# jnvance/DMRG.x

Hardware: NVIDIA B200
Metric: superblock H*psi algorithmic GB/s (higher is better)
Workload: dtype f64

## Files before the change

### dmrg.x_b200/csrc/abi.cpp

```cpp
#include <cstring>
#include <string>

#include "../../include/dmrgx.h"
#include <cmath>

#include "common.h"
#include "plan.h"

using namespace dmrgx;

namespace {
thread_local std::string g_msg;
template <class F>
int guard(F&& f) {
    try { f(); return 0; }
    catch (const Err& e) { g_msg = e.what(); return e.code ? e.code : 1; }
    catch (const std::exception& e) { g_msg = e.what(); return 1; }
    catch (...) { g_msg = "unknown error"; return 1; }
}
inline Ctx* cur(Ctx* c) { if (c && c->st) dev::make_current(c->st); return c; }
inline Ctx* C(dmrgx_ctx c) { return cur((Ctx*)c); }
inline Block* B(dmrgx_block b) { if (b) cur(((Block*)b)->ctx); return (Block*)b; }
inline Kron* K(dmrgx_kron k) { if (k) cur(((Kron*)k)->ctx); return (Kron*)k; }
inline HShell* H(dmrgx_hshell h) { if (h) cur(((HShell*)h)->ctx); return (HShell*)h; }
// ... 107 lines not shown
    *out = nullptr;
    return guard([&] { *out = (dmrgx_hshell)hshell_create(K(k), terms_of(nterms, a, iop, isite, jop, jsite)); });
}
int dmrgx_hshell_create_single(dmrgx_kron k, int opl, dmrgx_int il, int opr, dmrgx_int ir, dmrgx_hshell* out) {
    *out = nullptr;
    return guard([&] { *out = (dmrgx_hshell)hshell_create_single(K(k), opl, (int)il, opr, (int)ir); });
}
int dmrgx_hshell_create_product(dmrgx_kron k, dmrgx_int nl, const int* lop, const dmrgx_int* lsite, dmrgx_int nr, const int* rop,
                                const dmrgx_int* rsite, dmrgx_hshell* out) {
    *out = nullptr;
    return guard([&] {
        std::vector<std::pair<int, int>> l, r;
        for (dmrgx_int i = 0; i < nl; ++i) l.push_back({lop[i], (int)lsite[i]});
        for (dmrgx_int i = 0; i < nr; ++i) r.push_back({rop[i], (int)rsite[i]});
        *out = (dmrgx_hshell)hshell_create_product(K(k), l, r);
    });
}
int dmrgx_hshell_apply(dmrgx_hshell h, const double* d_x, double* d_y) { return guard([&] { hshell_apply(H(h), d_x, d_y); }); }
int dmrgx_hshell_apply_sharded(dmrgx_hshell h, double* d_x, double* d_y) { return guard([&] { hshell_apply_sharded(H(h), d_x, d_y); }); }
int dmrgx_hshell_halo_bytes(dmrgx_hshell h, double* halo, double* allgather) {
    HShell* s = H(h);
    if (halo) *halo = 8.0 * (double)s->halo_recv_elems;
    if (allgather) *allgather = 8.0 * (double)(s->n - (s->row_end - s->row_begin)) * (s->ctx->world > 1 ? 1.0 : 0.0);
    return 0;
}
int dmrgx_hshell_row_range(dmrgx_hshell h, dmrgx_int* begin, dmrgx_int* end, dmrgx_int* cuts) {
    HShell* s = H(h);
    if (begin) *begin = s->row_begin;
    if (end) *end = s->row_end;
    if (cuts) for (size_t i = 0; i < s->row_cuts.size(); ++i) cuts[i] = s->row_cuts[i];
    return 0;
}
int dmrgx_hshell_apply_stage(dmrgx_hshell h, int stage, const double* d_x, double* d_y) {
    return guard([&] {
        HShell* s = H(h);
        if (s->sparse) { if (stage == 2) hshell_apply(s, d_x, d_y); else if (stage != 1) throw Err(ERR_ARG_WRONG, "stage must be 1 or 2"); return; }
        if (stage == 1) s->stage1.run(s->ctx, d_x, nullptr);
        else if (stage == 2) s->stage2.run(s->ctx, d_x, d_y);
        else throw Err(ERR_ARG_WRONG, "stage must be 1 or 2");
    });
}
int dmrgx_hshell_stage_flops(dmrgx_hshell h, double* flops1, double* flops2) {
    *flops1 = H(h)->stage1.flops; *flops2 = H(h)->stage2.flops;
    return 0;
}
dmrgx_int dmrgx_hshell_plan_items(dmrgx_hshell h, int stage, dmrgx_int cap, dmrgx_int* out4) {
    const Plan& p = stage == 1 ? H(h)->stage1 : H(h)->stage2;
    dmrgx_int n = 0;
    for (const dev::WorkItem& it : p.items) {
        if (n < cap) {
            long long ks = 0;
            for (int sgi = it.seg_begin; sgi < it.seg_end; ++sgi) if (p.segs[sgi].type == dev::SEG_GEMM) ks += p.segs[sgi].K;
            out4[4 * n] = it.tm; out4[4 * n + 1] = it.tn; out4[4 * n + 2] = it.seg_end - it.seg_begin; out4[4 * n + 3] = ks;
        }
        ++n;
    }
    return n;
}
int dmrgx_hshell_plan_segtypes(dmrgx_hshell h, int stage, dmrgx_int* out6) {
    const Plan& p = stage == 1 ? H(h)->stage1 : H(h)->stage2;
    for (int i = 0; i < 6; ++i) out6[i] = 0;
    for (const dev::WorkItem& it : p.items)
        for (int sgi = it.seg_begin; sgi < it.seg_end; ++sgi) out6[p.segs[sgi].type]++;
    return 0;
}
int dmrgx_hshell_stage_exec_flops(dmrgx_hshell h, double* flops1, double* flops2) {
    *flops1 = H(h)->stage1.exec_flops; *flops2 = H(h)->stage2.exec_flops;
    return 0;
}
int dmrgx_hshell_apply_host(dmrgx_hshell h, const double* x, double* y) {
    return guard([&] {
        HShell* s = H(h);
        Ctx* ctx = s->ctx;
        const size_t bytes = (size_t)s->n * 8;
        if (!s->xbuf) {
            s->xbuf = std::make_shared<DevBuf>(ctx, bytes);
            s->ybuf = std::make_shared<DevBuf>(ctx, bytes);
        }
        const size_t lbytes = (size_t)(s->row_end - s->row_begin) * 8;
        dev::h2d(ctx->st, s->xbuf->as<double>() + s->row_begin, x, lbytes);
        hshell_apply_sharded(s, s->xbuf->as<double>(), s->ybuf->as<double>());
        dev::d2h(ctx->st, y, s->ybuf->as<double>() + s->row_begin, lbytes);
        dev::sync(ctx->st);
    });
}
int dmrgx_hshell_destroy(dmrgx_hshell h) { return guard([&] { if (h) { dev::sync(H(h)->ctx->st); delete H(h); } }); }
int dmrgx_hshell_workspace_bytes(dmrgx_hshell h, double* bytes) {
    HShell* s = H(h);
    double b = 16.0 * (double)s->n + (s->work ? (double)s->work->bytes : 0.0);
    for (const BufRef& k : s->keep) b += (double)k->bytes;
    *bytes = b;
    return 0;
}
int dmrgx_hshell_stats_global(dmrgx_hshell h, double* alg_bytes, double* alg_flops) {
    *alg_bytes = (double)H(h)->alg_bytes_global; *alg_flops = H(h)->alg_flops_global;
    return 0;
}
int dmrgx_hshell_stats(dmrgx_hshell h, dmrgx_int* nstates, dmrgx_int* nterms, double* alg_bytes, double* alg_flops, dmrgx_int* nt1, dmrgx_int* nt2) {
    HShell* s = H(h);
    if (nstates) *nstates = s->n;
    if (nterms) *nterms = s->nterms;
    if (alg_bytes) *alg_bytes = (double)s->alg_bytes;
    if (alg_flops) *alg_flops = s->alg_flops;
    if (nt1) *nt1 = (dmrgx_int)s->stage1.items.size();
    if (nt2) *nt2 = s->sparse ? (dmrgx_int)s->sparse->tiles.size() : (dmrgx_int)s->stage2.items.size();
    return 0;
// ... 201 lines not shown
```

### dmrg.x_b200/csrc/dev.h

```cpp
#pragma once
#include <cstddef>
#include <cstdint>

namespace dev {

enum SegType : int { SEG_GEMM = 0, SEG_AXPY = 1, SEG_DIAG = 2, SEG_CSRA = 3, SEG_CSRB = 4, SEG_CSRADD = 5 };

struct Segment {
    const double* A;
    const double* B;
    const int* rowptr;
    const int* colidx;
    long long lda_m, lda_k;
    long long ldb_n, ldb_k;
    double coef;
    int K;
    int type;
    int row0;
    int d;
    int flags;
    int pad;
};
enum : int { SEGF_A_X = 1, SEGF_B_X = 2 };

struct WorkItem {
    double* C;
    long long ldc;
    int m0, n0;
    int tm, tn;
    int seg_begin, seg_end;
    int mode;
    int c_in_y;
};

constexpr int TILE = 64;

struct Stream;

int init(int device, void* user_stream, Stream** out);
void destroy(Stream*);
const char* last_error();
void make_current(Stream*);

void* malloc_bytes(Stream*, size_t bytes);
void free_bytes(Stream*, void* p);
void h2d(Stream*, void* dst, const void* src, size_t bytes);
void d2h(Stream*, void* dst, const void* src, size_t bytes);
void d2d(Stream*, void* dst, const void* src, size_t bytes);
void memset0(Stream*, void* dst, size_t bytes);
void sync(Stream*);
long long launch_count();

constexpr int COMM_ID_BYTES = 128;
int comm_unique_id(void* out);
int comm_init(Stream*, int rank, int world, const void* id);
void allreduce_sum(Stream*, double* d_buf, long long n);
void allgatherv(Stream*, double* d_buf, const long long* offsets);
void exchange_ranges(Stream*, double* d_buf, int n, const int* from, const int* to, const long long* off, const long long* cnt);
void bcast_batch(Stream*, int n, double* const* d_ptr, const long long* count, const int* root);

void run_chain(Stream*, const WorkItem* d_items, int nitems, const Segment* d_segs, const double* x, double* y, double* w = nullptr);

constexpr int SP_ROWS = 4;
struct SpASlot { long long src[SP_ROWS]; double w[SP_ROWS]; };
struct SpSSlot { int roff[SP_ROWS]; int pad[SP_ROWS]; double w[SP_ROWS]; };
struct SpBSlot { const int* ecol; const double* eval; int W, ld; int all_in, pad; int roff[SP_ROWS]; long long src[SP_ROWS]; double w[SP_ROWS]; };
struct SpTile {
    long long off;
    int nR, nrows;
    int a_begin, a_count;
    int s_begin, s_count;
    int b_begin, b_count;
    int pad[6];
};
constexpr int SP_MAX_NR = 3072;
void run_spmm(Stream*, const SpTile* d_tiles, int ntiles, const SpASlot* d_aslots, const SpSSlot* d_sslots, const SpBSlot* d_bslots, const double* x, double* y,
              int max_nR);

struct ReduceItem {
    double* dst;
    long long ldc;
    long long src_off;
    int tm, tn;
    int nparts;
    int dst_in_y;
};
void run_reduce(Stream*, const ReduceItem* d_items, int nitems, double* y, const double* w);

// ... 18 lines not shown
```

### dmrg.x_b200/csrc/dev_cuda.cu

```cuda
#include <cuda_runtime.h>
#include <dlfcn.h>
#include <nccl.h>

#include <chrono>
#include <map>
#include <unordered_map>
#include <cstdio>
#include <cstring>
#include <algorithm>
#include <stdexcept>
#include <string>
#include <vector>

#include "dev.h"

namespace dev {

static thread_local std::string g_err;
static long long g_launches = 0;
const char* last_error() { return g_err.c_str(); }
long long launch_count() { return g_launches; }

#define CUDA_OK(call)                                                                                   \
    do {                                                                                                \
// ... 175 lines not shown
}

template <bool MK>
struct Stager {
    const double* base;
    int off[8];
    long long kstep;
    int soff;
    int k0;
    unsigned rowmask;
    static constexpr int SI = MK ? 8 * S_MK : 2 * S_KM;
    __device__ __forceinline__ void init(const double* b, long long ld_row, long long ld_k, int ext, int tid) {
        base = b;
        if (MK) {
            const int k = tid & 15, r0 = tid >> 4;
            rowmask = 0;
#pragma unroll
            for (int i = 0; i < 8; ++i) {
                int r = r0 + 8 * i;
                if (r < ext) rowmask |= 1u << i;
                r = r < ext ? r : ext - 1;
                off[i] = (int)(r * ld_row + k * ld_k);
            }
            soff = r0 * S_MK + k;
            k0 = k;
        } else {
            const int r = tid & 63, kk = tid >> 6;
            const int rc = r < ext ? r : ext - 1;
            rowmask = r < ext ? 0xffu : 0u;
#pragma unroll
            for (int i = 0; i < 8; ++i) off[i] = (int)(rc * ld_row + (kk + 2 * i) * ld_k);
            soff = kk * S_KM + r;
            k0 = kk;
        }
        kstep = (long long)BK * ld_k;
    }
    template <bool ALLROWS>
    __device__ __forceinline__ void issue(double* sm, int krem) {
        if (krem >= BK) {
#pragma unroll
            for (int i = 0; i < 8; ++i)
                if (ALLROWS || ((rowmask >> i) & 1u)) cp_async8_all(sm + soff + i * SI, base + off[i]);
        } else {
#pragma unroll
            for (int i = 0; i < 8; ++i) {
                const bool v = (MK ? k0 : k0 + 2 * i) < krem;
                if (ALLROWS || ((rowmask >> i) & 1u)) cp_async8(sm + soff + i * SI, v ? base + off[i] : base, v);
            }
        }
        base += kstep;
    }
};

template <bool A_MK, bool B_NK, bool UNIT, int NMI, int NNI, int NKK = BK / 4>
__device__ __forceinline__ void chunk_mma(double (&acc)[4][4][2], const double* as, const double* bs, double coef) {
    constexpr int a_sm = A_MK ? S_MK : 1, a_sk = A_MK ? 1 : S_KM;
    constexpr int b_sn = B_NK ? S_MK : 1, b_sk = B_NK ? 1 : S_KM;
#pragma unroll
    for (int kk = 0; kk < NKK; ++kk) {
        double a[NMI], b[NNI];
#pragma unroll
        for (int mi = 0; mi < NMI; ++mi) a[mi] = as[mi * 8 * a_sm + kk * 4 * a_sk];
#pragma unroll
        for (int ni = 0; ni < NNI; ++ni) b[ni] = UNIT ? bs[ni * 8 * b_sn + kk * 4 * b_sk] : bs[ni * 8 * b_sn + kk * 4 * b_sk] * coef;
#pragma unroll
        for (int ni = 0; ni < NNI; ++ni)
#pragma unroll
            for (int mi = 0; mi < NMI; ++mi) dmma_m8n8k4(acc[mi][ni][0], acc[mi][ni][1], a[mi], b[ni]);
    }
}

template <int NSTAGE, bool A_MK, bool B_NK, bool FULL, bool UNIT>
__device__ __forceinline__ void gemm_segment(double (&acc)[4][4][2], const Segment& sg, const WorkItem& it, double* As, double* Bs,
                                             int tid, int rbase, int cbase, int g, int t, int nmi, int nni) {
    Stager<A_MK> sa;
    Stager<B_NK> sb;
    sa.init(sg.A + (long long)it.m0 * sg.lda_m, sg.lda_m, sg.lda_k, it.tm, tid);
    sb.init(sg.B + (long long)it.n0 * sg.ldb_n, sg.ldb_n, sg.ldb_k, it.tn, tid);
    const int K = sg.K;
    const int nchunks = (K + BK - 1) / BK;
    const double coef = sg.coef;
    constexpr int a_sm = A_MK ? S_MK : 1, a_sk = A_MK ? 1 : S_KM;
    constexpr int b_sn = B_NK ? S_MK : 1, b_sk = B_NK ? 1 : S_KM;
    const int a_base = (rbase + g) * a_sm + t * a_sk;
    const int b_base = (cbase + g) * b_sn + t * b_sk;
    __syncthreads();
#pragma unroll
    for (int p = 0; p < NSTAGE - 1; ++p) {
        if (p < nchunks) {
            sa.template issue<FULL>(As + p * SMEM_TILE, K - p * BK);
            sb.template issue<FULL>(Bs + p * SMEM_TILE, K - p * BK);
        }
        cp_async_commit();
    }
    int cur = 0, nxt = NSTAGE - 1;
    for (int c = 0; c < nchunks; ++c) {
        if (c + NSTAGE - 1 < nchunks) {
            const int krem = K - (c + NSTAGE - 1) * BK;
            sa.template issue<FULL>(As + nxt * SMEM_TILE, krem);
            sb.template issue<FULL>(Bs + nxt * SMEM_TILE, krem);
        }
        cp_async_commit();
        cp_async_wait<NSTAGE - 1>();
        __syncthreads();
        const double* as = As + cur * SMEM_TILE + a_base;
        const double* bs = Bs + cur * SMEM_TILE + b_base;
        if (FULL) {
            const int krem = K - c * BK;
            if (krem > 12) chunk_mma<A_MK, B_NK, UNIT, 4, 4, 4>(acc, as, bs, coef);
            else if (krem > 8) chunk_mma<A_MK, B_NK, UNIT, 4, 4, 3>(acc, as, bs, coef);
            else if (krem > 4) chunk_mma<A_MK, B_NK, UNIT, 4, 4, 2>(acc, as, bs, coef);
            else chunk_mma<A_MK, B_NK, UNIT, 4, 4, 1>(acc, as, bs, coef);
        } else {
#define MMA_CASE(M_, N_) case (M_) * 5 + (N_): chunk_mma<A_MK, B_NK, UNIT, M_, N_>(acc, as, bs, coef); break;
            switch (nmi * 5 + nni) {
                MMA_CASE(4, 4) MMA_CASE(4, 3) MMA_CASE(4, 2) MMA_CASE(4, 1)
                MMA_CASE(3, 4) MMA_CASE(3, 3) MMA_CASE(3, 2) MMA_CASE(3, 1)
                MMA_CASE(2, 4) MMA_CASE(2, 3) MMA_CASE(2, 2) MMA_CASE(2, 1)
                MMA_CASE(1, 4) MMA_CASE(1, 3) MMA_CASE(1, 2) MMA_CASE(1, 1)
                default: break;
            }
#undef MMA_CASE
        }
        __syncthreads();
        cur = cur + 1 == NSTAGE ? 0 : cur + 1;
        nxt = nxt + 1 == NSTAGE ? 0 : nxt + 1;
    }
}

template <int NSTAGE, bool A_MK, bool B_NK>
__device__ __forceinline__ void gemm_dispatch(double (&acc)[4][4][2], const Segment& sg, const WorkItem& it, double* As, double* Bs,
                                              int tid, int rbase, int cbase, int g, int t, int nmi, int nni) {
    if (sg.coef == 1.0) {
        if (it.tm == BM && it.tn == BM) gemm_segment<NSTAGE, A_MK, B_NK, true, true>(acc, sg, it, As, Bs, tid, rbase, cbase, g, t, 4, 4);
        else gemm_segment<NSTAGE, A_MK, B_NK, false, true>(acc, sg, it, As, Bs, tid, rbase, cbase, g, t, nmi, nni);
    } else gemm_segment<NSTAGE, A_MK, B_NK, false, false>(acc, sg, it, As, Bs, tid, rbase, cbase, g, t, nmi, nni);
}

template <int NSTAGE>
__global__ void __launch_bounds__(NTHREADS, 3) chain_kernel(const WorkItem* __restrict__ items, const Segment* __restrict__ segs,
                                                            const double* __restrict__ xbase, double* __restrict__ ybase,
                                                            double* __restrict__ wbase) {
    extern __shared__ __align__(16) double chain_smem[];
    double* As = chain_smem;
    double* Bs = chain_smem + NSTAGE * SMEM_TILE;
    WorkItem it = items[blockIdx.x];
    if (it.c_in_y) it.C = (double*)((char*)(it.c_in_y == 1 ? ybase : wbase) + (size_t)it.C);
    const int tid = threadIdx.x;
    const int warp = tid >> 5, lane = tid & 31;
    const int wm = warp >> 1, wn = warp & 1;
    const int g = lane >> 2, t = lane & 3;
    const int tm = it.tm, tn = it.tn;
    const int hm = ((tm + 15) >> 4) << 3, hn = ((tn + 15) >> 4) << 3;
    const int rbase = wm * hm, cbase = wn * hn;
    int nmi = (tm - rbase + 7) / 8; nmi = nmi < 0 ? 0 : (nmi > (hm >> 3) ? (hm >> 3) : nmi);
    int nni = (tn - cbase + 7) / 8; nni = nni < 0 ? 0 : (nni > (hn >> 3) ? (hn >> 3) : nni);

    double acc[4][4][2];
#pragma unroll
    for (int mi = 0; mi < 4; ++mi)
#pragma unroll
        for (int ni = 0; ni < 4; ++ni) { acc[mi][ni][0] = 0.0; acc[mi][ni][1] = 0.0; }

    for (int s = it.seg_begin; s < it.seg_end; ++s) {
        Segment sg = segs[s];
        if (sg.flags & SEGF_A_X) sg.A = (const double*)((const char*)xbase + (size_t)sg.A);
        if (sg.flags & SEGF_B_X) sg.B = (const double*)((const char*)xbase + (size_t)sg.B);
        if (sg.type == SEG_GEMM) {
            const bool a_mk = (sg.lda_k == 1) || (sg.lda_m != 1);
            const bool b_nk = (sg.ldb_k == 1) || (sg.ldb_n != 1);
            if (a_mk) {
                if (b_nk) gemm_dispatch<NSTAGE, true, true>(acc, sg, it, As, Bs, tid, rbase, cbase, g, t, nmi, nni);
                else gemm_dispatch<NSTAGE, true, false>(acc, sg, it, As, Bs, tid, rbase, cbase, g, t, nmi, nni);
            } else {
                if (b_nk) gemm_dispatch<NSTAGE, false, true>(acc, sg, it, As, Bs, tid, rbase, cbase, g, t, nmi, nni);
                else gemm_dispatch<NSTAGE, false, false>(acc, sg, it, As, Bs, tid, rbase, cbase, g, t, nmi, nni);
            }
        } else if (sg.type == SEG_AXPY) {
            const double* base = sg.A + (long long)(it.m0 + rbase + g) * sg.lda_m + (long long)(it.n0 + cbase + 2 * t) * sg.lda_k;
            const long long sm8 = 8 * sg.lda_m, sn8 = 8 * sg.lda_k, sn1 = sg.lda_k;
            double v[4][4][2];
#pragma unroll
            for (int mi = 0; mi < 4; ++mi) {
                const bool rok = mi < nmi && rbase + mi * 8 + g < tm;
#pragma unroll
                for (int ni = 0; ni < 4; ++ni) {
                    const int col = cbase + ni * 8 + 2 * t;
                    const bool c0 = rok && ni < nni && col < tn, c1 = rok && ni < nni && col + 1 < tn;
                    const double* q = base + mi * sm8 + ni * sn8;
                    v[mi][ni][0] = c0 ? q[0] : 0.0;
                    v[mi][ni][1] = c1 ? q[sn1] : 0.0;
                }
            }
            const double coef = sg.coef;
#pragma unroll
            for (int mi = 0; mi < 4; ++mi)
#pragma unroll
                for (int ni = 0; ni < 4; ++ni) { acc[mi][ni][0] += coef * v[mi][ni][0]; acc[mi][ni][1] += coef * v[mi][ni][1]; }
        } else if (sg.type == SEG_CSRA) {
            const double* xb = sg.A + (long long)(it.n0 + cbase + 2 * t) * sg.ldb_n;
#pragma unroll
            for (int mi = 0; mi < 4; ++mi) {
                const int row = rbase + mi * 8 + g;
                if (mi >= nmi || row >= tm) continue;
                const int r = sg.row0 + it.m0 + row;
                const int e1 = sg.rowptr[r + 1];
                for (int e = sg.rowptr[r]; e < e1; ++e) {
                    const double v = sg.B[e] * sg.coef;
                    const double* xr = xb + (long long)sg.colidx[e] * sg.ldb_k;
// ... 7 lines not shown
            }
        } else if (sg.type == SEG_CSRB) {
            const double* vb = sg.A + (long long)(it.m0 + rbase + g) * sg.lda_m;
#pragma unroll
            for (int ni = 0; ni < 4; ++ni) {
#pragma unroll
                for (int h = 0; h < 2; ++h) {
                    const int col = cbase + ni * 8 + 2 * t + h;
                    if (ni >= nni || col >= tn) continue;
                    const int r = sg.row0 + it.n0 + col;
                    const int e1 = sg.rowptr[r + 1];
                    for (int e = sg.rowptr[r]; e < e1; ++e) {
                        const double v = sg.B[e] * sg.coef;
                        const double* vc = vb + (long long)sg.colidx[e] * sg.lda_k;
#pragma unroll
                        for (int mi = 0; mi < 4; ++mi)
                            if (mi < nmi && rbase + mi * 8 + g < tm) acc[mi][ni][h] += v * vc[(long long)(mi * 8) * sg.lda_m];
                    }
                }
            }
        } else if (sg.type == SEG_CSRADD) {
#pragma unroll
            for (int mi = 0; mi < 4; ++mi) {
                const int row = rbase + mi * 8 + g;
                if (mi >= nmi || row >= tm) continue;
                const int r = sg.row0 + it.m0 + row;
                const int e1 = sg.rowptr[r + 1];
                for (int e = sg.rowptr[r]; e < e1; ++e) {
                    const int lc = sg.colidx[e] - sg.d - it.n0 - cbase - 2 * t;
                    const double v = sg.B[e] * sg.coef;
#pragma unroll
                    for (int ni = 0; ni < 4; ++ni) {
                        const int col = cbase + ni * 8 + 2 * t;
                        if (ni < nni && lc == ni * 8 && col < tn) acc[mi][ni][0] += v;
                        if (ni < nni && lc == ni * 8 + 1 && col + 1 < tn) acc[mi][ni][1] += v;
                    }
                }
            }
        } else if (sg.type == SEG_DIAG) {
#pragma unroll
            for (int mi = 0; mi < 4; ++mi) {
                const int row = rbase + mi * 8 + g;
                if (mi >= nmi || row >= tm) continue;
#pragma unroll
                for (int ni = 0; ni < 4; ++ni)
#pragma unroll
                    for (int h = 0; h < 2; ++h) {
                        const int col = cbase + ni * 8 + 2 * t + h;
                        if (ni < nni && col < tn && it.m0 + row + sg.d == it.n0 + col) acc[mi][ni][h] += sg.coef;
                    }
            }
        }
    }
#pragma unroll
    for (int mi = 0; mi < 4; ++mi) {
        const int row = rbase + mi * 8 + g;
        if (mi >= nmi || row >= tm) continue;
#pragma unroll
        for (int ni = 0; ni < 4; ++ni) {
#pragma unroll
            for (int h = 0; h < 2; ++h) {
                const int col = cbase + ni * 8 + 2 * t + h;
                if (ni >= nni || col >= tn) continue;
                double* p = it.C + (long long)row * it.ldc + col;
                if (it.mode == 0) *p = acc[mi][ni][h];
                else atomicAdd(p, acc[mi][ni][h]);
            }
        }
    }
}

void run_chain(Stream* st, const WorkItem* d_items, int nitems, const Segment* d_segs, const double* x, double* y, double* w) {
    if (nitems <= 0) return;
    constexpr int smem2 = 2 * 2 * SMEM_TILE * (int)sizeof(double), smem3 = 2 * 3 * SMEM_TILE * (int)sizeof(double);
    if (!st->chain_cfg) {
        CUDA_OK(cudaFuncSetAttribute(chain_kernel<3>, cudaFuncAttributeMaxDynamicSharedMemorySize, smem3));
        st->chain_cfg = true;
    }
    constexpr int deep_below = 1800;
    if (nitems < deep_below) chain_kernel<3><<<nitems, NTHREADS, smem3, st->s>>>(d_items, d_segs, x, y, w);
    else chain_kernel<2><<<nitems, NTHREADS, smem2, st->s>>>(d_items, d_segs, x, y, w);
    LAUNCH_CHECK();
}

constexpr int SP_BD = 256, SP_CH = 4, SP_AMAX = 24, SP_BMAX = 8;

__device__ __forceinline__ unsigned smem_u32(const void* p) { return (unsigned)__cvta_generic_to_shared(p); }
__device__ __forceinline__ void mbar_init(unsigned long long* b, int count) {
    asm volatile("mbarrier.init.shared::cta.b64 [%0], %1;\n" ::"r"(smem_u32(b)), "r"(count));
    asm volatile("fence.mbarrier_init.release.cluster;\n" ::: "memory");
}
__device__ __forceinline__ void mbar_expect_tx(unsigned long long* b, unsigned bytes) {
    asm volatile("mbarrier.arrive.expect_tx.shared::cta.b64 _, [%0], %1;\n" ::"r"(smem_u32(b)), "r"(bytes) : "memory");
}
__device__ __forceinline__ void bulk_g2s(void* dst, const void* src, unsigned bytes, unsigned long long* b) {
    asm volatile("cp.async.bulk.shared::cluster.global.mbarrier::complete_tx::bytes [%0], [%1], %2, [%3];\n" ::"r"(smem_u32(dst)), "l"(src), "r"(bytes),
                 "r"(smem_u32(b))
                 : "memory");
}
__device__ __forceinline__ void mbar_wait(unsigned long long* b, unsigned parity) {
    unsigned ok;
    do {
        asm volatile("{\n.reg .pred p;\nmbarrier.try_wait.parity.shared::cta.b64 p, [%1], %2;\nselp.u32 %0, 1, 0, p;\n}\n" : "=r"(ok) : "r"(smem_u32(b)), "r"(parity) : "memory");
    } while (!ok);
}

template <class T>
__device__ __forceinline__ void sp_stage(T* dst, const T* src, int count, int tid) {
    for (int i = tid; i < count * (int)(sizeof(T) / 8); i += SP_BD) ((double*)dst)[i] = __ldg((const double*)src + i);
}

__global__ void __launch_bounds__(SP_BD, 3) spmm_kernel(const SpTile* __restrict__ tiles, const SpASlot* __restrict__ aslots, const SpSSlot* __restrict__ sslots,
                                                       const SpBSlot* __restrict__ bslots, const double* __restrict__ x, double* __restrict__ y) {
    extern __shared__ __align__(16) unsigned char sp_smem[];
    __shared__ unsigned long long mbar;
    __shared__ SpTile s_tile;
// ... 1118 lines not shown
    const int max_sweeps = 40;
    while (!live.empty()) {
        const int nl = (int)live.size();
        int* sub_prefix = h_tab.data();
        int* app_prefix = h_tab.data() + nl + 1;
        sub_prefix[0] = 0; app_prefix[0] = 0;
        int maxnb = 0;
        for (int q = 0; q < nl; ++q) {
            const EigJob& jb = jobs[(size_t)live[(size_t)q]];
            ljobs[(size_t)q] = jb;
            const int npair = jb.nb / 2;
            sub_prefix[q + 1] = sub_prefix[q] + npair;
            app_prefix[q + 1] = app_prefix[q] + npair * (npair - 1) / 2 + npair * (jb.np / ET);
            maxnb = std::max(maxnb, jb.nb);
        }
        CUDA_OK(cudaMemcpyAsync(d_live, ljobs.data(), (size_t)nl * sizeof(EigJob), cudaMemcpyHostToDevice, st->s));
        CUDA_OK(cudaMemcpyAsync(d_tab, h_tab.data(), (size_t)(2 * nl + 2) * 4, cudaMemcpyHostToDevice, st->s));
        CUDA_OK(cudaStreamSynchronize(st->s));
        for (int rr = 0; rr < maxnb - 1; ++rr, ++round) {
            eig_sub_kernel<<<sub_prefix[nl], ESUB_THREADS, sub_smem, st->s>>>(d_live, d_tab, nl, round, sweeps_done == 0);
            LAUNCH_CHECK();
            eig_apply_kernel<<<app_prefix[nl], 128, app_smem, st->s>>>(d_live, d_tab + nl + 1, nl, round);
            LAUNCH_CHECK();
        }
        ++sweeps_done;
        for (int q = 0; q < nl; ++q) CUDA_OK(cudaMemcpyAsync(&h_active[(size_t)q], jobs[(size_t)live[(size_t)q]].active, 4, cudaMemcpyDeviceToHost, st->s));
        CUDA_OK(cudaStreamSynchronize(st->s));
        std::vector<int> next;
        for (int q = 0; q < nl; ++q) if (h_active[(size_t)q]) next.push_back(live[(size_t)q]);
        for (int q : next) CUDA_OK(cudaMemsetAsync(jobs[(size_t)q].active, 0, 4, st->s));
        live.swap(next);
        if (round > max_sweeps * 256 || (round / std::max(1, maxnb - 1)) > max_sweeps) { if (!live.empty()) { g_err = "block Jacobi did not converge"; rc = 107; } break; }
    }
    WorkItem* d_items = nullptr;
    Segment* d_segs = nullptr;
    if (!rc) {
        std::vector<WorkItem> items;
        std::vector<Segment> segs;
        for (int q = 0; q < nj; ++q) {
            const EigJob& jb = jobs[(size_t)q];
            Segment sg;
            std::memset(&sg, 0, sizeof sg);
            sg.type = SEG_GEMM; sg.coef = 1.0; sg.K = jb.n;
            sg.A = jb.VT; sg.lda_m = jb.np; sg.lda_k = 1;
            sg.B = jb.outA; sg.ldb_n = 1; sg.ldb_k = jb.n;
            segs.push_back(sg);
            for (int m0 = 0; m0 < jb.n; m0 += TILE)
                for (int n0 = 0; n0 < jb.n; n0 += TILE) {
                    WorkItem it;
                    std::memset(&it, 0, sizeof it);
                    it.C = jb.A + (long long)m0 * jb.np + n0; it.ldc = jb.np; it.m0 = m0; it.n0 = n0;
                    it.tm = std::min(TILE, jb.n - m0); it.tn = std::min(TILE, jb.n - n0);
                    it.seg_begin = q; it.seg_end = q + 1;
                    items.push_back(it);
                }
        }
        d_items = (WorkItem*)malloc_bytes(st, items.size() * sizeof(WorkItem));
        d_segs = (Segment*)malloc_bytes(st, segs.size() * sizeof(Segment));
        CUDA_OK(cudaMemcpyAsync(d_items, items.data(), items.size() * sizeof(WorkItem), cudaMemcpyHostToDevice, st->s));
        CUDA_OK(cudaMemcpyAsync(d_segs, segs.data(), segs.size() * sizeof(Segment), cudaMemcpyHostToDevice, st->s));
        for (int q = 0; q < nj; ++q) h_tab[(size_t)q] = (int)lam_off[(size_t)q];
        CUDA_OK(cudaMemcpyAsync(d_tab, rank_off.data(), (size_t)nj * 4, cudaMemcpyHostToDevice, st->s));
        CUDA_OK(cudaMemcpyAsync(d_tab + nj, h_tab.data(), (size_t)nj * 4, cudaMemcpyHostToDevice, st->s));
        run_chain(st, d_items, (int)items.size(), d_segs, nullptr, nullptr, nullptr);
        eig_rq_kernel<<<dim3(16, nj), 256, 0, st->s>>>(d_jobs, wd, d_tab + nj);
        LAUNCH_CHECK();
        eig_finish_kernel<<<dim3(4, nj), 256, 0, st->s>>>(d_jobs, wd, d_tab + nj, wi, d_tab);
        LAUNCH_CHECK();
        eig_gather_kernel<<<dim3(64, nj), 256, 0, st->s>>>(d_jobs, wi, d_tab);
        LAUNCH_CHECK();
        CUDA_OK(cudaStreamSynchronize(st->s));
    }
    join();
    CUDA_OK(cudaStreamSynchronize(st->s));
    free_bytes(st, d_items);
    free_bytes(st, d_segs);
    free_bytes(st, d_live);
    free_bytes(st, d_jobs);
    free_bytes(st, wi);
    free_bytes(st, wd);
    return rc;
}

}
```

### dmrg.x_b200/csrc/plan.cpp

```cpp
#include <algorithm>
#include <cmath>
#include <chrono>
#include <cstdio>
#include <cstdlib>
#include <cstring>

#include "common.h"
#include "plan.h"

namespace dmrgx {

bool Trace::enabled() { static const bool on = getenv("DMRGX_TRACE") != nullptr; return on; }
double Trace::now() { return std::chrono::duration<double>(std::chrono::steady_clock::now().time_since_epoch()).count(); }
Trace::Trace(Ctx* c, const char* w) : ctx(c), what(w), t0(0), on(enabled()) { if (on) { dev::sync(ctx->st); t0 = now(); } }
void Trace::mark(const char* label) {
    if (!on) return;
    dev::sync(ctx->st);
    const double t = now();
    fprintf(stderr, "[trace] %s.%s %.3f ms\n", what, label, (t - t0) * 1e3);
    t0 = t;
}

void Plan::upload(Ctx* ctx) {
    if (items.empty()) return;
    std::vector<double> cost(items.size());
    for (size_t i = 0; i < items.size(); ++i) {
        double c = 0;
        for (int s = items[i].seg_begin; s < items[i].seg_end; ++s) c += segs[s].type == dev::SEG_GEMM ? (double)segs[s].K : 1.0;
        cost[i] = c * items[i].tm * items[i].tn + 64.0;
    }
    std::vector<size_t> ord(items.size());
    for (size_t i = 0; i < ord.size(); ++i) ord[i] = i;
    const bool by_phase = item_phase.size() == items.size();
    std::stable_sort(ord.begin(), ord.end(), [&](size_t a, size_t b) {
        if (by_phase && item_phase[a] != item_phase[b]) return item_phase[a] < item_phase[b];
        return cost[a] > cost[b];
    });
    std::vector<dev::WorkItem> sorted(items.size());
    for (size_t i = 0; i < ord.size(); ++i) sorted[i] = items[ord[i]];
    items.swap(sorted);
    d_items = std::make_shared<DevBuf>(ctx, items.size() * sizeof(dev::WorkItem));
    d_segs = std::make_shared<DevBuf>(ctx, std::max<size_t>(1, segs.size()) * sizeof(dev::Segment));
    dev::h2d(ctx->st, d_items->p, items.data(), items.size() * sizeof(dev::WorkItem));
    dev::h2d(ctx->st, d_segs->p, segs.data(), segs.size() * sizeof(dev::Segment));
    if (!reduces.empty()) {
        d_reduces = std::make_shared<DevBuf>(ctx, reduces.size() * sizeof(dev::ReduceItem));
        dev::h2d(ctx->st, d_reduces->p, reduces.data(), reduces.size() * sizeof(dev::ReduceItem));
        scratch = std::make_shared<DevBuf>(ctx, (size_t)scratch_elems * 8);
    }
    dev::sync(ctx->st);
}

void Plan::run(Ctx* ctx, const double* x, double* y) const {
    if (items.empty()) return;
    double* w = scratch ? scratch->as<double>() : nullptr;
    dev::run_chain(ctx->st, d_items->as<dev::WorkItem>(), (int)items.size(), d_segs->as<dev::Segment>(), x, y, w);
    if (!reduces.empty()) dev::run_reduce(ctx->st, d_reduces->as<dev::ReduceItem>(), (int)reduces.size(), y, w);
}

static inline const double* padd(const double* p, long long elems) { return p + elems; }

void emit_cells(Plan& plan, double* C, bool c_in_y, long long ldc, int R, int Ncols, const std::vector<Contribution>& contribs,
                bool cover_all) {
    if (R <= 0 || Ncols <= 0) return;
    std::vector<int> rc = {0, R}, cc = {0, Ncols};
    for (const Contribution& c : contribs) {
        if (c.nr <= 0 || c.nc <= 0) continue;
        if (c.r0 < 0 || c.c0 < 0 || c.r0 + c.nr > R || c.c0 + c.nc > Ncols) throw Err(ERR_GENERIC, "emit_cells: contribution outside the panel");
        rc.push_back(c.r0); rc.push_back(c.r0 + c.nr);
        cc.push_back(c.c0); cc.push_back(c.c0 + c.nc);
    }
    std::sort(rc.begin(), rc.end()); rc.erase(std::unique(rc.begin(), rc.end()), rc.end());
    std::sort(cc.begin(), cc.end()); cc.erase(std::unique(cc.begin(), cc.end()), cc.end());
    for (size_t ri = 0; ri + 1 < rc.size(); ++ri) {
        const int r0 = rc[ri], r1 = rc[ri + 1];
        for (size_t ci = 0; ci + 1 < cc.size(); ++ci) {
            const int c0 = cc[ci], c1 = cc[ci + 1];
            const int seg_begin = (int)plan.segs.size();
            double kflops = 0;
            for (const Contribution& c : contribs) {
                if (c.nr <= 0 || c.nc <= 0) continue;
                if (!(c.r0 <= r0 && r1 <= c.r0 + c.nr && c.c0 <= c0 && c1 <= c.c0 + c.nc)) continue;
                dev::Segment s = c.seg;
                const long long dr = r0 - c.r0, dc = c0 - c.c0;
                switch (s.type) {
                    case dev::SEG_GEMM: s.A = padd(s.A, dr * s.lda_m); s.B = padd(s.B, dc * s.ldb_n); kflops += 2.0 * s.K; break;
                    case dev::SEG_AXPY: s.A = padd(s.A, dr * s.lda_m + dc * s.lda_k); break;
                    case dev::SEG_DIAG: s.d = (int)(s.d + dr - dc); break;
                    case dev::SEG_CSRA: s.row0 += (int)dr; s.A = padd(s.A, dc * s.ldb_n); break;
                    case dev::SEG_CSRB: s.row0 += (int)dc; s.A = padd(s.A, dr * s.lda_m); break;
                    case dev::SEG_CSRADD: s.row0 += (int)dr; s.d = (int)(s.d + dc); break;
                    default: throw Err(ERR_GENERIC, "emit_cells: bad segment type");
                }
                plan.segs.push_back(s);
            }
            const int seg_end = (int)plan.segs.size();
            if (seg_end == seg_begin && !cover_all) continue;
            const int M = r1 - r0, N = c1 - c0;
            auto split = [](int len) {
                std::vector<int> ext;
                const int nfull = len / 64, rem = len % 64;
                for (int i = 0; i < nfull; ++i) ext.push_back(64);
                if (rem == 0) return ext;
                if (nfull > 0 && rem < 24) {
                    ext.pop_back();
                    const int tot = 64 + rem, h = (((tot + 1) / 2) + 7) / 8 * 8;
                    ext.push_back(h); ext.push_back(tot - h);
                } else ext.push_back(rem);
                return ext;
            };
            const std::vector<int> em = split(M), en = split(N);
            std::vector<int> part_begin = {seg_begin};
            if (plan.split_item_cost > 0 && seg_end - seg_begin > 1) {
                double ktot = 0;
                for (int sgi = seg_begin; sgi < seg_end; ++sgi) ktot += plan.segs[sgi].type == dev::SEG_GEMM ? plan.segs[sgi].K : 0;
                const double area = (double)em[0] * (double)en[0];
                int nparts = (int)std::ceil(ktot * area / plan.split_item_cost);
                nparts = std::max(1, std::min(nparts, seg_end - seg_begin));
                if (nparts > 1) {
                    double acc = 0;
                    int next = 1;
                    for (int sgi = seg_begin; sgi < seg_end && next < nparts; ++sgi) {
                        acc += plan.segs[sgi].type == dev::SEG_GEMM ? plan.segs[sgi].K : 0;
                        if (acc >= ktot * next / nparts && sgi + 1 < seg_end) { part_begin.push_back(sgi + 1); ++next; }
                    }
                }
            }
            part_begin.push_back(seg_end);
            const int nparts = (int)part_begin.size() - 1;
            int m0 = 0;
            for (int tm : em) {
                int n0 = 0;
                for (int tn : en) {
                    dev::WorkItem it;
                    std::memset(&it, 0, sizeof it);
                    it.m0 = m0; it.n0 = n0;
                    it.tm = tm; it.tn = tn;
                    it.mode = 0;
                    double* dst = C + (long long)(r0 + m0) * ldc + (c0 + n0);
                    {
                        auto frag = [](int t) { const int h = ((t + 15) >> 4) << 3; const int a = std::min(h, ((t + 7) / 8) * 8);
                                                const int b = std::max(0, std::min(h, ((t - h + 7) / 8) * 8)); return a + b; };
                        double kx = 0;
                        for (int sgi = seg_begin; sgi < seg_end; ++sgi)
                            if (plan.segs[sgi].type == dev::SEG_GEMM) kx += 16.0 * ((plan.segs[sgi].K + 15) / 16);
                        plan.exec_flops += 2.0 * frag(tm) * frag(tn) * kx;
                    }
                    if (nparts == 1) {
                        it.C = dst; it.ldc = ldc; it.c_in_y = c_in_y ? 1 : 0;
                        it.seg_begin = seg_begin; it.seg_end = seg_end;
                        plan.items.push_back(it);
                        plan.item_phase.push_back(0);
                    } else {
                        dev::ReduceItem ri;
                        std::memset(&ri, 0, sizeof ri);
                        ri.dst = dst; ri.ldc = ldc; ri.dst_in_y = c_in_y ? 1 : 0;
                        ri.src_off = plan.scratch_elems * 8; ri.tm = tm; ri.tn = tn; ri.nparts = nparts;
                        plan.reduces.push_back(ri);
                        for (int pp = 0; pp < nparts; ++pp) {
                            it.C = (double*)(uintptr_t)((plan.scratch_elems + (long long)pp * tm * tn) * 8);
                            it.ldc = tn; it.c_in_y = 2;
                            it.seg_begin = part_begin[pp]; it.seg_end = part_begin[pp + 1];
                            plan.items.push_back(it);
                            plan.item_phase.push_back(pp);
                        }
                        plan.scratch_elems += (long long)nparts * tm * tn;
                    }
                    n0 += tn;
                }
                m0 += tm;
            }
            plan.flops += kflops * (double)M * (double)N;
        }
    }
}

}
```

### include/dmrgx.h

```cpp
#ifndef DMRGX_H
#define DMRGX_H

#ifdef __cplusplus
extern "C" {
#endif

typedef long long dmrgx_int;

typedef struct dmrgx_ctx_s* dmrgx_ctx;
typedef struct dmrgx_block_s* dmrgx_block;
typedef struct dmrgx_kron_s* dmrgx_kron;
typedef struct dmrgx_hshell_s* dmrgx_hshell;
typedef struct dmrgx_xform_s* dmrgx_xform;

enum { DMRGX_OP_SM = -1, DMRGX_OP_SZ = 0, DMRGX_OP_SP = 1, DMRGX_OP_EYE = 2, DMRGX_OP_H = 3 };

const char* dmrgx_last_error(void);
dmrgx_int dmrgx_launch_count(void);

int dmrgx_ctx_create(int device, void* stream, dmrgx_ctx* out);
int dmrgx_dist_unique_id(void* out128);
int dmrgx_ctx_create_dist(int device, void* stream, int rank, int world, const void* id128, dmrgx_ctx* out);
int dmrgx_ctx_rank(dmrgx_ctx ctx, int* rank, int* world);
int dmrgx_ctx_destroy(dmrgx_ctx ctx);
int dmrgx_ctx_sync(dmrgx_ctx ctx);
int dmrgx_ctx_set_dense_threshold(dmrgx_ctx ctx, double fill);

int dmrgx_block_create(dmrgx_ctx ctx, dmrgx_int nsites, dmrgx_int nsectors, const double* qn_list, const dmrgx_int* qn_size,
                       dmrgx_block* out);
int dmrgx_block_single_site(dmrgx_ctx ctx, int spin_twice, dmrgx_block* out);
int dmrgx_block_set_operator(dmrgx_block blk, int op, dmrgx_int isite, const dmrgx_int* rowptr, const dmrgx_int* colidx,
                             const double* values);
int dmrgx_block_get_operator(dmrgx_block blk, int op, dmrgx_int isite, dmrgx_int* nnz, dmrgx_int* rowptr, dmrgx_int* colidx,
                             double* values);
int dmrgx_block_info(dmrgx_block blk, dmrgx_int* nsites, dmrgx_int* nstates, dmrgx_int* nsectors);
int dmrgx_block_sectors(dmrgx_block blk, double* qn_list, dmrgx_int* qn_size);
int dmrgx_block_check(dmrgx_block blk);
int dmrgx_block_destroy(dmrgx_block blk);
int dmrgx_block_enlarge(dmrgx_block left, dmrgx_block site, dmrgx_int nterms, const double* a, const int* iop, const dmrgx_int* isite,
                        const int* jop, const dmrgx_int* jsite, dmrgx_block* out);

int dmrgx_kron_create(dmrgx_block left, dmrgx_block right, dmrgx_int nqn, const double* qn_sectors, dmrgx_kron* out);
int dmrgx_kron_destroy(dmrgx_kron k);
dmrgx_int dmrgx_kron_size(dmrgx_kron k);
dmrgx_int dmrgx_kron_num_states(dmrgx_kron k);
int dmrgx_kron_data(dmrgx_kron k, double* qn, dmrgx_int* left_idx, dmrgx_int* right_idx, dmrgx_int* sizes, dmrgx_int* offsets);
dmrgx_int dmrgx_kron_map(dmrgx_kron k, dmrgx_int lidx, dmrgx_int ridx);
dmrgx_int dmrgx_kron_offsets_lr(dmrgx_kron k, dmrgx_int lidx, dmrgx_int ridx);

int dmrgx_hshell_create(dmrgx_kron k, dmrgx_int nterms, const double* a, const int* iop, const dmrgx_int* isite, const int* jop,
                        const dmrgx_int* jsite, dmrgx_hshell* out);
int dmrgx_hshell_create_single(dmrgx_kron k, int op_left, dmrgx_int isite_left, int op_right, dmrgx_int isite_right, dmrgx_hshell* out);
int dmrgx_hshell_create_product(dmrgx_kron k, dmrgx_int nl, const int* lop, const dmrgx_int* lsite, dmrgx_int nr, const int* rop,
                                const dmrgx_int* rsite, dmrgx_hshell* out);
int dmrgx_hshell_apply(dmrgx_hshell h, const double* d_x, double* d_y);
int dmrgx_hshell_apply_sharded(dmrgx_hshell h, double* d_x, double* d_y);
int dmrgx_hshell_halo_bytes(dmrgx_hshell h, double* halo_recv_bytes, double* allgather_recv_bytes);
int dmrgx_hshell_row_range(dmrgx_hshell h, dmrgx_int* begin, dmrgx_int* end, dmrgx_int* cuts);
int dmrgx_hshell_apply_stage(dmrgx_hshell h, int stage, const double* d_x, double* d_y);
int dmrgx_hshell_stage_flops(dmrgx_hshell h, double* flops_stage1, double* flops_stage2);
int dmrgx_hshell_stage_exec_flops(dmrgx_hshell h, double* flops_stage1, double* flops_stage2);
int dmrgx_hshell_plan_segtypes(dmrgx_hshell h, int stage, dmrgx_int* out6);
dmrgx_int dmrgx_hshell_plan_items(dmrgx_hshell h, int stage, dmrgx_int cap, dmrgx_int* out4);
int dmrgx_hshell_apply_host(dmrgx_hshell h, const double* x, double* y);
int dmrgx_hshell_destroy(dmrgx_hshell h);
int dmrgx_hshell_stats(dmrgx_hshell h, dmrgx_int* nstates, dmrgx_int* nterms, double* alg_bytes, double* alg_flops,
                       dmrgx_int* ntiles_stage1, dmrgx_int* ntiles_stage2);

int dmrgx_hshell_workspace_bytes(dmrgx_hshell h, double* bytes);
int dmrgx_hshell_stats_global(dmrgx_hshell h, double* alg_bytes, double* alg_flops);

typedef struct {
    double tol;
    dmrgx_int ncv;
    dmrgx_int max_it;
    unsigned long long seed;
} dmrgx_eigs_opts;
typedef struct { dmrgx_int nmatvec, nrestart, converged; double resid; } dmrgx_eigs_stats;
int dmrgx_eigs_smallest(dmrgx_hshell h, const dmrgx_eigs_opts* opts, double* e0, double* d_psi, dmrgx_eigs_stats* stats);
int dmrgx_eigs_smallest_from(dmrgx_hshell h, const dmrgx_eigs_opts* opts, const double* d_initial, double* e0, double* d_psi, dmrgx_eigs_stats* stats);

typedef struct dmrgx_wave_s* dmrgx_wave;
int dmrgx_wave_create(dmrgx_kron k, const double* d_psi, dmrgx_xform grown_side, int grow_left, dmrgx_wave* out);
int dmrgx_wave_apply(dmrgx_wave w, dmrgx_xform shrinking_side, dmrgx_block site, dmrgx_kron k_new, double* d_psi_new, int* ok);
int dmrgx_wave_destroy(dmrgx_wave w);

int dmrgx_truncate(dmrgx_kron k, const double* d_psi, dmrgx_int mstates, dmrgx_xform* left, dmrgx_xform* right);
int dmrgx_xform_info(dmrgx_xform x, dmrgx_int* m, dmrgx_int* nstates, dmrgx_int* nsectors, double* trunc_err, dmrgx_int* nspectrum);
int dmrgx_xform_sectors(dmrgx_xform x, double* qn_list, dmrgx_int* qn_size);
int dmrgx_xform_spectrum(dmrgx_xform x, double* eigval, dmrgx_int* blk_idx);
int dmrgx_xform_rotmat(dmrgx_xform x, double* out);
int dmrgx_xform_destroy(dmrgx_xform x);

int dmrgx_rotate(dmrgx_block enlarged, dmrgx_xform x, dmrgx_block* out);

int dmrgx_expect(dmrgx_hshell h1, const double* d_psi, double* value);

int dmrgx_corr_matrix(dmrgx_kron k, const double* d_psi, double* szsz, double* spsm, double* smsp, double* sz, double* flops);

int dmrgx_dimer_matrix(dmrgx_kron k, const double* d_psi, dmrgx_int nbonds, const dmrgx_int* site_i, const dmrgx_int* site_j, double* dd,
                       double* d, double* flops);

dmrgx_int dmrgx_ham_terms(dmrgx_int Lx, dmrgx_int Ly, double J1, double Jz1, double J2, double Jz2, int bcx, int bcy, dmrgx_int nsites,
                          dmrgx_int maxterms, double* a, int* iop, dmrgx_int* isite, int* jop, dmrgx_int* jsite);

int dmrgx_selftest_gemm(dmrgx_ctx ctx, dmrgx_int M, dmrgx_int N, dmrgx_int K, int a_k_contig, int b_k_contig, int nseg, int reps, double* ms,
                        double* max_err);

int dmrgx_selftest_eig(dmrgx_ctx ctx, dmrgx_int nblocks, const dmrgx_int* n, double* a, double* w, double* ms);

int dmrgx_vec_alloc(dmrgx_ctx ctx, dmrgx_int n, double** d_out);
int dmrgx_vec_free(dmrgx_ctx ctx, double* d);
int dmrgx_vec_set(dmrgx_ctx ctx, double* d_dst, const double* h_src, dmrgx_int n);
int dmrgx_vec_get(dmrgx_ctx ctx, double* h_dst, const double* d_src, dmrgx_int n);

#ifdef __cplusplus
// ... 4 lines not shown
```

Measured before the change: 65.28.

## Choose per-tile warp split for skinny GEMM tiles and interleave edge tiles in schedule

Each work item now carries a warp layout (2x2, 1x4 or 4x1) and per-warp fragment counts chosen on the host to minimise the largest per-warp fragment count for skinny edge tiles. The kernel maps fragments into the fixed accumulator array through slot remapping and writes back accordingly. Non-unit coefficients on partial tiles are now applied by scaling the B shared tile in place instead of per-fragment multiplies. The scheduler also interleaves edge tiles among full tiles outside the last waves to balance load. This adds template instantiations and register pressure, and an extra syncthreads on scaled partial tiles.

```diff
diff --git a/dmrg.x_b200/csrc/abi.cpp b/dmrg.x_b200/csrc/abi.cpp
--- a/dmrg.x_b200/csrc/abi.cpp
+++ b/dmrg.x_b200/csrc/abi.cpp
@@ -183,6 +183,18 @@
             long long ks = 0;
             for (int sgi = it.seg_begin; sgi < it.seg_end; ++sgi) if (p.segs[sgi].type == dev::SEG_GEMM) ks += p.segs[sgi].K;
             out4[4 * n] = it.tm; out4[4 * n + 1] = it.tn; out4[4 * n + 2] = it.seg_end - it.seg_begin; out4[4 * n + 3] = ks;
+        }
+        ++n;
+    }
+    return n;
+}
+dmrgx_int dmrgx_hshell_plan_warps(dmrgx_hshell h, int stage, dmrgx_int cap, dmrgx_int* out9) {
+    const Plan& p = stage == 1 ? H(h)->stage1 : H(h)->stage2;
+    dmrgx_int n = 0;
+    for (const dev::WorkItem& it : p.items) {
+        if (n < cap) {
+            out9[9 * n] = it.warps;
+            for (int w = 0; w < 4; ++w) { out9[9 * n + 1 + 2 * w] = (it.frags >> (8 * w)) & 15; out9[9 * n + 2 + 2 * w] = (it.frags >> (8 * w + 4)) & 15; }
         }
         ++n;
     }
diff --git a/dmrg.x_b200/csrc/dev.h b/dmrg.x_b200/csrc/dev.h
--- a/dmrg.x_b200/csrc/dev.h
+++ b/dmrg.x_b200/csrc/dev.h
@@ -1,4 +1,5 @@
 #pragma once
+#include <algorithm>
 #include <cstddef>
 #include <cstdint>
 
@@ -31,9 +32,30 @@
     int seg_begin, seg_end;
     int mode;
     int c_in_y;
+    int warps;
+    unsigned frags;
 };
+enum : int { WARPS_2X2 = 0, WARPS_1X4 = 1, WARPS_4X1 = 2 };
 
 constexpr int TILE = 64;
+
+inline void set_warp_split(WorkItem& it, bool gemm_only) {
+    const int fm = (it.tm + 7) / 8, fn = (it.tn + 7) / 8;
+    const int cost22 = ((fm + 1) / 2) * ((fn + 1) / 2), cost14 = fm * ((fn + 3) / 4), cost41 = ((fm + 3) / 4) * fn;
+    int split = WARPS_2X2;
+    if (gemm_only && cost14 < cost22 && cost14 <= cost41) split = WARPS_1X4;
+    else if (gemm_only && cost41 < cost22) split = WARPS_4X1;
+    const int qm = split == WARPS_2X2 ? (fm + 1) / 2 : split == WARPS_1X4 ? fm : (fm + 3) / 4;
+    const int qn = split == WARPS_2X2 ? (fn + 1) / 2 : split == WARPS_1X4 ? (fn + 3) / 4 : fn;
+    it.warps = split;
+    it.frags = 0;
+    for (int w = 0; w < 4; ++w) {
+        const int wr = split == WARPS_2X2 ? w >> 1 : split == WARPS_1X4 ? 0 : w;
+        const int wc = split == WARPS_2X2 ? w & 1 : split == WARPS_1X4 ? w : 0;
+        const int nm = std::max(0, std::min(qm, fm - wr * qm)), nn = std::max(0, std::min(qn, fn - wc * qn));
+        it.frags |= (unsigned)(nm | nn << 4) << (8 * w);
+    }
+}
 
 struct Stream;
 
diff --git a/dmrg.x_b200/csrc/dev_cuda.cu b/dmrg.x_b200/csrc/dev_cuda.cu
--- a/dmrg.x_b200/csrc/dev_cuda.cu
+++ b/dmrg.x_b200/csrc/dev_cuda.cu
@@ -251,25 +251,31 @@
     }
 };
 
-template <bool A_MK, bool B_NK, bool UNIT, int NMI, int NNI, int NKK = BK / 4>
-__device__ __forceinline__ void chunk_mma(double (&acc)[4][4][2], const double* as, const double* bs, double coef) {
+template <int NMI, int NNI> __device__ __forceinline__ constexpr int slot_i(int mi, int ni) { return NMI > 4 ? (mi & 3) : NNI > 4 ? mi + 2 * (ni >> 2) : mi; }
+template <int NMI, int NNI> __device__ __forceinline__ constexpr int slot_j(int mi, int ni) { return NMI > 4 ? ni + 2 * (mi >> 2) : NNI > 4 ? (ni & 3) : ni; }
+
+template <bool A_MK, bool B_NK, int NMI, int NNI, int NKK = BK / 4>
+__device__ __forceinline__ void chunk_mma(double (&acc)[4][4][2], const double* as, const double* bs) {
     constexpr int a_sm = A_MK ? S_MK : 1, a_sk = A_MK ? 1 : S_KM;
     constexpr int b_sn = B_NK ? S_MK : 1, b_sk = B_NK ? 1 : S_KM;
 #pragma unroll
     for (int kk = 0; kk < NKK; ++kk) {
-        double a[NMI], b[NNI];
+        double a[NMI > 0 ? NMI : 1], b[NNI > 0 ? NNI : 1];
 #pragma unroll
         for (int mi = 0; mi < NMI; ++mi) a[mi] = as[mi * 8 * a_sm + kk * 4 * a_sk];
 #pragma unroll
-        for (int ni = 0; ni < NNI; ++ni) b[ni] = UNIT ? bs[ni * 8 * b_sn + kk * 4 * b_sk] : bs[ni * 8 * b_sn + kk * 4 * b_sk] * coef;
+        for (int ni = 0; ni < NNI; ++ni) b[ni] = bs[ni * 8 * b_sn + kk * 4 * b_sk];
 #pragma unroll
         for (int ni = 0; ni < NNI; ++ni)
 #pragma unroll
-            for (int mi = 0; mi < NMI; ++mi) dmma_m8n8k4(acc[mi][ni][0], acc[mi][ni][1], a[mi], b[ni]);
-    }
-}
-
-template <int NSTAGE, bool A_MK, bool B_NK, bool FULL, bool UNIT>
+            for (int mi = 0; mi < NMI; ++mi) {
+                double (&c)[2] = acc[slot_i<NMI, NNI>(mi, ni)][slot_j<NMI, NNI>(mi, ni)];
+                dmma_m8n8k4(c[0], c[1], a[mi], b[ni]);
+            }
+    }
+}
+
+template <int NSTAGE, bool A_MK, bool B_NK, bool FULL>
 __device__ __forceinline__ void gemm_segment(double (&acc)[4][4][2], const Segment& sg, const WorkItem& it, double* As, double* Bs,
                                              int tid, int rbase, int cbase, int g, int t, int nmi, int nni) {
     Stager<A_MK> sa;
@@ -306,17 +312,24 @@
         const double* bs = Bs + cur * SMEM_TILE + b_base;
         if (FULL) {
             const int krem = K - c * BK;
-            if (krem > 12) chunk_mma<A_MK, B_NK, UNIT, 4, 4, 4>(acc, as, bs, coef);
-            else if (krem > 8) chunk_mma<A_MK, B_NK, UNIT, 4, 4, 3>(acc, as, bs, coef);
-            else if (krem > 4) chunk_mma<A_MK, B_NK, UNIT, 4, 4, 2>(acc, as, bs, coef);
-            else chunk_mma<A_MK, B_NK, UNIT, 4, 4, 1>(acc, as, bs, coef);
+            if (krem > 12) chunk_mma<A_MK, B_NK, 4, 4, 4>(acc, as, bs);
+            else if (krem > 8) chunk_mma<A_MK, B_NK, 4, 4, 3>(acc, as, bs);
+            else if (krem > 4) chunk_mma<A_MK, B_NK, 4, 4, 2>(acc, as, bs);
+            else chunk_mma<A_MK, B_NK, 4, 4, 1>(acc, as, bs);
         } else {
-#define MMA_CASE(M_, N_) case (M_) * 5 + (N_): chunk_mma<A_MK, B_NK, UNIT, M_, N_>(acc, as, bs, coef); break;
-            switch (nmi * 5 + nni) {
+            if (coef != 1.0) {
+                double* bst = Bs + cur * SMEM_TILE;
+                for (int i = tid; i < SMEM_TILE; i += NTHREADS) bst[i] *= coef;
+                __syncthreads();
+            }
+#define MMA_CASE(M_, N_) case (M_) * 9 + (N_): chunk_mma<A_MK, B_NK, M_, N_>(acc, as, bs); break;
+            switch (nmi * 9 + nni) {
                 MMA_CASE(4, 4) MMA_CASE(4, 3) MMA_CASE(4, 2) MMA_CASE(4, 1)
                 MMA_CASE(3, 4) MMA_CASE(3, 3) MMA_CASE(3, 2) MMA_CASE(3, 1)
                 MMA_CASE(2, 4) MMA_CASE(2, 3) MMA_CASE(2, 2) MMA_CASE(2, 1)
                 MMA_CASE(1, 4) MMA_CASE(1, 3) MMA_CASE(1, 2) MMA_CASE(1, 1)
+                MMA_CASE(7, 2) MMA_CASE(7, 1) MMA_CASE(5, 2) MMA_CASE(5, 1)
+                MMA_CASE(2, 7) MMA_CASE(1, 7) MMA_CASE(2, 5) MMA_CASE(1, 5)
                 default: break;
             }
 #undef MMA_CASE
@@ -330,10 +343,8 @@
 template <int NSTAGE, bool A_MK, bool B_NK>
 __device__ __forceinline__ void gemm_dispatch(double (&acc)[4][4][2], const Segment& sg, const WorkItem& it, double* As, double* Bs,
                                               int tid, int rbase, int cbase, int g, int t, int nmi, int nni) {
-    if (sg.coef == 1.0) {
-        if (it.tm == BM && it.tn == BM) gemm_segment<NSTAGE, A_MK, B_NK, true, true>(acc, sg, it, As, Bs, tid, rbase, cbase, g, t, 4, 4);
-        else gemm_segment<NSTAGE, A_MK, B_NK, false, true>(acc, sg, it, As, Bs, tid, rbase, cbase, g, t, nmi, nni);
-    } else gemm_segment<NSTAGE, A_MK, B_NK, false, false>(acc, sg, it, As, Bs, tid, rbase, cbase, g, t, nmi, nni);
+    if (sg.coef == 1.0 && it.tm == BM && it.tn == BM) gemm_segment<NSTAGE, A_MK, B_NK, true>(acc, sg, it, As, Bs, tid, rbase, cbase, g, t, 4, 4);
+    else gemm_segment<NSTAGE, A_MK, B_NK, false>(acc, sg, it, As, Bs, tid, rbase, cbase, g, t, nmi, nni);
 }
 
 template <int NSTAGE>
@@ -347,13 +358,14 @@
     if (it.c_in_y) it.C = (double*)((char*)(it.c_in_y == 1 ? ybase : wbase) + (size_t)it.C);
     const int tid = threadIdx.x;
     const int warp = tid >> 5, lane = tid & 31;
-    const int wm = warp >> 1, wn = warp & 1;
     const int g = lane >> 2, t = lane & 3;
     const int tm = it.tm, tn = it.tn;
-    const int hm = ((tm + 15) >> 4) << 3, hn = ((tn + 15) >> 4) << 3;
-    const int rbase = wm * hm, cbase = wn * hn;
-    int nmi = (tm - rbase + 7) / 8; nmi = nmi < 0 ? 0 : (nmi > (hm >> 3) ? (hm >> 3) : nmi);
-    int nni = (tn - cbase + 7) / 8; nni = nni < 0 ? 0 : (nni > (hn >> 3) ? (hn >> 3) : nni);
+    const int split = it.warps;
+    const unsigned frags = it.frags;
+    const int nmi = (frags >> (8 * warp)) & 15, nni = (frags >> (8 * warp + 4)) & 15;
+    const int wr = split == WARPS_2X2 ? warp >> 1 : split == WARPS_1X4 ? 0 : warp;
+    const int wc = split == WARPS_2X2 ? warp & 1 : split == WARPS_1X4 ? warp : 0;
+    const int rbase = wr * 8 * (int)(frags & 15), cbase = wc * 8 * (int)((frags >> 4) & 15);
 
     double acc[4][4][2];
 #pragma unroll
@@ -467,16 +479,20 @@
             }
         }
     }
+    const int di = split == WARPS_4X1 ? 16 : 0, rj = split == WARPS_1X4 ? 32 : 0;
+    const int dj = split == WARPS_1X4 ? 16 : 0, ci = split == WARPS_4X1 ? 32 : 0;
 #pragma unroll
     for (int mi = 0; mi < 4; ++mi) {
-        const int row = rbase + mi * 8 + g;
-        if (mi >= nmi || row >= tm) continue;
 #pragma unroll
         for (int ni = 0; ni < 4; ++ni) {
+            const int ro = mi * 8 - (mi >= 2 ? di : 0) + (ni >= 2 ? rj : 0);
+            const int co = ni * 8 - (ni >= 2 ? dj : 0) + (mi >= 2 ? ci : 0);
+            const int row = rbase + ro + g;
+            if (ro >= 8 * nmi || co >= 8 * nni || row >= tm) continue;
 #pragma unroll
             for (int h = 0; h < 2; ++h) {
-                const int col = cbase + ni * 8 + 2 * t + h;
-                if (ni >= nni || col >= tn) continue;
+                const int col = cbase + co + 2 * t + h;
+                if (col >= tn) continue;
                 double* p = it.C + (long long)row * it.ldc + col;
                 if (it.mode == 0) *p = acc[mi][ni][h];
                 else atomicAdd(p, acc[mi][ni][h]);
@@ -1701,6 +1717,7 @@
                     it.C = jb.A + (long long)m0 * jb.np + n0; it.ldc = jb.np; it.m0 = m0; it.n0 = n0;
                     it.tm = std::min(TILE, jb.n - m0); it.tn = std::min(TILE, jb.n - n0);
                     it.seg_begin = q; it.seg_end = q + 1;
+                    set_warp_split(it, true);
                     items.push_back(it);
                 }
         }
diff --git a/dmrg.x_b200/csrc/plan.cpp b/dmrg.x_b200/csrc/plan.cpp
--- a/dmrg.x_b200/csrc/plan.cpp
+++ b/dmrg.x_b200/csrc/plan.cpp
@@ -36,6 +36,16 @@
         if (by_phase && item_phase[a] != item_phase[b]) return item_phase[a] < item_phase[b];
         return cost[a] > cost[b];
     });
+    constexpr size_t last_wave = 3 * 148;
+    const size_t head = ord.size() > last_wave ? ord.size() - last_wave : 0;
+    for (size_t b = 0, e; b < head; b = e) {
+        for (e = b + 1; e < head && (!by_phase || item_phase[ord[e]] == item_phase[ord[b]]); ++e) {}
+        std::vector<size_t> full, edge;
+        for (size_t i = b; i < e; ++i) (items[ord[i]].tm == dev::TILE && items[ord[i]].tn == dev::TILE ? full : edge).push_back(ord[i]);
+        const size_t len = e - b;
+        size_t ie = 0, jf = 0;
+        for (size_t p = 0; p < len; ++p) ord[b + p] = ie < (p + 1) * edge.size() / len ? edge[ie++] : full[jf++];
+    }
     std::vector<dev::WorkItem> sorted(items.size());
     for (size_t i = 0; i < ord.size(); ++i) sorted[i] = items[ord[i]];
     items.swap(sorted);
@@ -128,6 +138,10 @@
             }
             part_begin.push_back(seg_end);
             const int nparts = (int)part_begin.size() - 1;
+            auto gemm_only = [&](int b, int e) {
+                for (int sgi = b; sgi < e; ++sgi) if (plan.segs[sgi].type != dev::SEG_GEMM) return false;
+                return true;
+            };
             int m0 = 0;
             for (int tm : em) {
                 int n0 = 0;
@@ -149,6 +163,7 @@
                     if (nparts == 1) {
                         it.C = dst; it.ldc = ldc; it.c_in_y = c_in_y ? 1 : 0;
                         it.seg_begin = seg_begin; it.seg_end = seg_end;
+                        dev::set_warp_split(it, gemm_only(seg_begin, seg_end));
                         plan.items.push_back(it);
                         plan.item_phase.push_back(0);
                     } else {
@@ -161,6 +176,7 @@
                             it.C = (double*)(uintptr_t)((plan.scratch_elems + (long long)pp * tm * tn) * 8);
                             it.ldc = tn; it.c_in_y = 2;
                             it.seg_begin = part_begin[pp]; it.seg_end = part_begin[pp + 1];
+                            dev::set_warp_split(it, gemm_only(it.seg_begin, it.seg_end));
                             plan.items.push_back(it);
                             plan.item_phase.push_back(pp);
                         }
diff --git a/include/dmrgx.h b/include/dmrgx.h
--- a/include/dmrgx.h
+++ b/include/dmrgx.h
@@ -62,6 +62,7 @@
 int dmrgx_hshell_stage_exec_flops(dmrgx_hshell h, double* flops_stage1, double* flops_stage2);
 int dmrgx_hshell_plan_segtypes(dmrgx_hshell h, int stage, dmrgx_int* out6);
 dmrgx_int dmrgx_hshell_plan_items(dmrgx_hshell h, int stage, dmrgx_int cap, dmrgx_int* out4);
+dmrgx_int dmrgx_hshell_plan_warps(dmrgx_hshell h, int stage, dmrgx_int cap, dmrgx_int* out9);
 int dmrgx_hshell_apply_host(dmrgx_hshell h, const double* x, double* y);
 int dmrgx_hshell_destroy(dmrgx_hshell h);
 int dmrgx_hshell_stats(dmrgx_hshell h, dmrgx_int* nstates, dmrgx_int* nterms, double* alg_bytes, double* alg_flops,
```

After: 63.36, median of 6. 2.9% lower.
